# hypha-space/hypha

Hardware: AMD Instinct MI355X
Metric: tokens/sec (node) + outer-sync bytes, Llama-3-8B DiLoCo H=100 at 1/2/4/8 GPUs (higher is better)
Workload: dtype bf16; 1 GPU; model=llama3-8b, global_batch=8, seq_len=2048, parallelism=diloco-dp1, h=100, model_params=8030261248, memory_mode=full, outer_sync_payload_bytes=16060522496, outer_sync_wire_bytes_per_rank=0, comm_reduction_vs_ddp=100x fewer syncs, bf16 payload, native_ops=True

## Files before the change

hypha_amd/ops/hip/attention.hip:

```cpp

#include <climits>

#include <torch/extension.h>

#include "attn_tile.h"
#include "hip_common.h"

namespace {

typedef __attribute__((ext_vector_type(2))) __bf16 bf16x2;

template <int HD>
__global__ __launch_bounds__(256, 1) void attn_fwd_kernel(
    const short* __restrict__ qg, const short* __restrict__ kg,
    const short* __restrict__ vg, short* __restrict__ og, float* __restrict__ lseg,
    int B, int Hq, int Hkv, int S, float scale, bool causal,
    long long q_sb, long long q_sh, long long q_ss,
    long long kv_sb, long long kv_sh, long long kv_ss) {
  constexpr int KC = HD / 16;
  constexpr int DBLK = HD / 32;
  __shared__ __attribute__((aligned(16))) short k_lds[KVB * HD];
  __shared__ __attribute__((aligned(16))) short vt_lds[HD * VT_PITCH];
  __shared__ __attribute__((aligned(16))) short ot_lds[NWAVE][QB * (HD + 8)];

  const int tid = threadIdx.x;
  const int lane = tid & 63;
  const int wid = tid >> 6;
  const int hi = lane >> 5;
  const int ln = lane & 31;

  const int bh = blockIdx.y;
  const int b = bh / Hq;
  const int hq = bh % Hq;
  const int hkv = hq / (Hq / Hkv);
  const long long qbase = (long long)b * q_sb + (long long)hq * q_sh;
  const long long kvbase = (long long)b * kv_sb + (long long)hkv * kv_sh;

  const int q0wg = blockIdx.x * WGQ;
  const int q0 = q0wg + wid * QB;
  const int qrow = q0 + ln;
  const int vis = causal ? qrow : INT_MAX;

  s16x8 qfrag[KC];
// ... 58 lines not shown
    q_sh = HD; q_ss = (long long)Hq * HD; q_sb = (long long)S * Hq * HD;
    kv_sh = HD; kv_ss = (long long)Hkv * HD; kv_sb = (long long)S * Hkv * HD;
  } else {
    q_ss = HD; q_sh = (long long)S * HD; q_sb = (long long)Hq * S * HD;
    kv_ss = HD; kv_sh = (long long)S * HD; kv_sb = (long long)Hkv * S * HD;
  }
#define LAUNCH_FWD(HDV)                                                                 \
  hipLaunchKernelGGL(attn_fwd_kernel<HDV>, grid, dim3(256), 0, stream,                  \
                     (const short*)q.data_ptr(), (const short*)k.data_ptr(),            \
                     (const short*)v.data_ptr(), (short*)o.data_ptr(),                  \
                     lse.data_ptr<float>(), B, Hq, Hkv, S, scale, causal, q_sb, q_sh,   \
                     q_ss, kv_sb, kv_sh, kv_ss)
  if (HD == 128)
    LAUNCH_FWD(128);
  else
    LAUNCH_FWD(64);
#undef LAUNCH_FWD
  return {o, lse};
}

std::vector<torch::Tensor> attn_fwd(torch::Tensor q, torch::Tensor k, torch::Tensor v,
                                    bool causal) {
  return attn_fwd_ex(q, k, v, causal, "bhsd");
}


namespace {

template <int HD>
__global__ void attn_bwd_di_kernel(const short* __restrict__ dog,
                                   const short* __restrict__ og,
                                   float* __restrict__ dig, long long nrows, int Hq,
                                   int S, long long sb, long long sh, long long ss) {
  const long long row = (long long)blockIdx.x * 4 + (threadIdx.x >> 6);
  if (row >= nrows) return;
  const long long b = row / ((long long)Hq * S);
  const long long h = (row / S) % Hq;
  const long long sq = row % S;
  const long long addr = b * sb + h * sh + sq * ss;
  const int lane = threadIdx.x & 63;
  float acc = 0.f;
#pragma unroll
  for (int i = 0; i < HD / 64; ++i) {
    int d = lane + 64 * i;
    acc += bf2f(dog[addr + d]) * bf2f(og[addr + d]);
  }
  acc = wave_reduce_sum(acc);
  if (lane == 0) dig[row] = acc;
}

__global__ void cast_f32_to_bf16_kernel(const float* __restrict__ in,
                                        short* __restrict__ out, long long n) {
  const long long stride = (long long)gridDim.x * blockDim.x * 4;
  for (long long base = ((long long)blockIdx.x * blockDim.x + threadIdx.x) * 4; base < n;
       base += stride) {
    if (base + 4 <= n) {
      f32x4 v = *reinterpret_cast<const f32x4*>(in + base);
      s16x4 o;
#pragma unroll
      for (int j = 0; j < 4; ++j) o[j] = f2bf(v[j]);
      *reinterpret_cast<s16x4*>(out + base) = o;
    } else {
      for (long long i = base; i < n; ++i) out[i] = f2bf(in[i]);
    }
  }
}

template <int HD>
__global__ __launch_bounds__(256, 1) void attn_bwd_v4_kernel(
    const short* __restrict__ qg, const short* __restrict__ kg,
    const short* __restrict__ vg, const short* __restrict__ dog,
    const float* __restrict__ lseg, const float* __restrict__ dig,
    float* __restrict__ dqg, short* __restrict__ dkg, short* __restrict__ dvg,
    int B, int Hq, int Hkv, int S, float scale, bool causal,
    long long q_sb, long long q_sh, long long q_ss,
    long long kv_sb, long long kv_sh, long long kv_ss, int ablate,
    int dq_bf16) {
  constexpr int KVT = 32;
  constexpr int NT = 4;
  constexpr int KVW = NT * KVT;
  constexpr int QT = 32;
  constexpr int KC = HD / 16;
  constexpr int DBLK = HD / 32;
  constexpr int TP = 40;
  constexpr int DSP = KVW + 8;
  constexpr int KTP = KVW + 8;
  __shared__ __attribute__((aligned(16))) short k_img[KVW * HD];
  __shared__ __attribute__((aligned(16))) short v_img[KVW * HD];
  __shared__ __attribute__((aligned(16))) short kt_img[HD * KTP];
  __shared__ __attribute__((aligned(16))) short qt_img[HD * 32];
  __shared__ __attribute__((aligned(16))) short dot_img[HD * 32];
  __shared__ __attribute__((aligned(16))) short ptds_img[NWAVE][KVT * TP];
  __shared__ __attribute__((aligned(16))) short dst_img[NWAVE][KVT * TP];
  __shared__ __attribute__((aligned(16))) short ds_img[2][QT * DSP];

  const int tid = threadIdx.x;
  const int lane = tid & 63;
  const int wid = tid >> 6;
  const int hi = lane >> 5;
  const int ln = lane & 31;

  const int bhkv = blockIdx.y;
  const int b = bhkv / Hkv;
  const int hkv = bhkv % Hkv;
  const int G = Hq / Hkv;
  const int kv_base = blockIdx.x * KVW;
  const long long kvbase = (long long)b * kv_sb + (long long)hkv * kv_sh;

  auto qimg_off = [](int d, int qe) {
    return d * 32 + ((((qe >> 3) ^ ((d >> 2) & 3)) << 3) | (qe & 7));
  };

  {
    constexpr int CH = KVW * HD / 8;
    for (int c = tid; c < CH; c += 256) {
      int row = c / (HD / 8), e0 = (c % (HD / 8)) * 8;
      s16x8 k8 = *reinterpret_cast<const s16x8*>(kg + kvbase + (long long)(kv_base + row) * kv_ss + e0);
      *reinterpret_cast<s16x8*>((char*)k_img + k_lds_off<HD>(row, e0)) = k8;
      s16x8 v8 = *reinterpret_cast<const s16x8*>(vg + kvbase + (long long)(kv_base + row) * kv_ss + e0);
      *reinterpret_cast<s16x8*>((char*)v_img + k_lds_off<HD>(row, e0)) = v8;
    }
#pragma unroll
    for (int half = 0; half < KVW / 64; ++half) {
      for (int i = 0; i < HD / 32; ++i) {
        int kvr = (tid & 63) + 64 * half;
        int e0 = (i * 4 + (tid >> 6)) * 8;
        s16x8 k8 = *reinterpret_cast<const s16x8*>(kg + kvbase + (long long)(kv_base + kvr) * kv_ss + e0);
#pragma unroll
        for (int j = 0; j < 8; ++j) kt_img[(e0 + j) * KTP + kvr] = k8[j];
      }
    }
  }
  __syncthreads();

  f32x16 dk_acc[DBLK] = {};
  f32x16 dv_acc[DBLK] = {};

  short* ptds = ptds_img[wid];
  short* dst = dst_img[wid];
  const int kv0 = kv_base + wid * KVT;

  const int t0 = causal ? kv_base / QT : 0;
  const int Tq = S / QT;
  constexpr int NSTG = HD / 16 / NWAVE;

  int prev_q0 = -1, prev_na = 0, pbuf = 0;
  long long prev_qbase = 0;

  auto run_dq = [&](int buf) {
    if (wid >= DBLK || prev_q0 < 0) return;
    const int db = wid;
    const int kck_hi = 2 * prev_na;
    f32x16 dq = {};
    for (int kck = 0; kck < kck_hi; ++kck) {
      s16x8 af = *reinterpret_cast<const s16x8*>(ds_img[buf] + ln * DSP + 16 * kck + 8 * hi);
      s16x8 bf = *reinterpret_cast<const s16x8*>(kt_img + (32 * db + ln) * KTP +
                                                 16 * kck + 8 * hi);
      dq = __builtin_amdgcn_mfma_f32_32x32x16_bf16(af, bf, dq, 0, 0, 0);
    }
    if (!(ablate & 1)) {
      if (dq_bf16) {
#pragma unroll
        for (int r = 0; r < 16; ++r) {
          int qi = prev_q0 + (r & 3) + 8 * (r >> 2) + 4 * hi;
          float other = __shfl_xor(dq[r], 1, 64);
          if ((ln & 1) == 0) {
            bf16x2 pkt;
            pkt.x = (__bf16)dq[r];
            pkt.y = (__bf16)other;
            __builtin_amdgcn_global_atomic_fadd_v2bf16(
                reinterpret_cast<bf16x2*>(
                    reinterpret_cast<short*>(dqg) +
                    (prev_qbase + (long long)qi * q_ss + 32 * db + ln)),
                pkt);
          }
        }
      } else {
#pragma unroll
        for (int r = 0; r < 16; ++r) {
          int qi = prev_q0 + (r & 3) + 8 * (r >> 2) + 4 * hi;
          atomicAdd(dqg + (prev_qbase + (long long)qi * q_ss + 32 * db + ln), dq[r]);
        }
      }
    } else {
      asm volatile("" ::"v"(dq[0]));
    }
  };

  for (int hq = hkv * G; hq < (hkv + 1) * G; ++hq) {
    const long long qbase = (long long)b * q_sb + (long long)hq * q_sh;
    const long long lsebase = (long long)(b * Hq + hq) * S;

    s16x8 qreg[NSTG], doreg[NSTG];
    auto issue_prefetch = [&](int t) {
#pragma unroll
      for (int i = 0; i < NSTG; ++i) {
        int it = wid + NWAVE * i;
        int d0 = 8 * hi + 16 * it;
        qreg[i] = *reinterpret_cast<const s16x8*>(qg + qbase + (long long)(t * QT + ln) * q_ss + d0);
        doreg[i] = *reinterpret_cast<const s16x8*>(dog + qbase + (long long)(t * QT + ln) * q_ss + d0);
      }
    };
    issue_prefetch(t0);
    float lse = lseg[lsebase + t0 * QT + ln];
    float di = dig[lsebase + t0 * QT + ln];

    for (int t = t0; t < Tq; ++t) {
      const int q0 = t * QT;
      const int qrow = q0 + ln;

#pragma unroll
      for (int i = 0; i < NSTG; ++i) {
        int it = wid + NWAVE * i;
        int d0 = 8 * hi + 16 * it;
#pragma unroll
        for (int j = 0; j < 8; ++j) {
          qt_img[qimg_off(d0 + j, ln)] = qreg[i][j];
          dot_img[qimg_off(d0 + j, ln)] = doreg[i][j];
        }
      }
      __syncthreads();

      const float lse_cur = lse, di_cur = di;
      if (t + 1 < Tq) {
        issue_prefetch(t + 1);
        lse = lseg[lsebase + (t + 1) * QT + ln];
        di = dig[lsebase + (t + 1) * QT + ln];
      }

      const int na = causal ? min(NT, (q0 + QT - 1 - kv_base) / KVT + 1) : NT;
      const int cbuf = pbuf ^ 1;

      if (!(ablate & 2)) run_dq(pbuf);

      if (wid < na) {
        f32x16 st = {};
#pragma unroll
        for (int kc = 0; kc < KC; ++kc) {
          s16x8 qf = *reinterpret_cast<const s16x8*>(qg + qbase + (long long)qrow * q_ss +
                                                     16 * kc + 8 * hi);
          s16x8 kf = *reinterpret_cast<const s16x8*>(
              (char*)k_img + k_lds_off<HD>(wid * KVT + ln, 16 * kc + 8 * hi));
          st = __builtin_amdgcn_mfma_f32_32x32x16_bf16(kf, qf, st, 0, 0, 0);
        }
        f32x16 pt;
#pragma unroll
        for (int r = 0; r < 16; ++r) {
          int kv = kv0 + (r & 3) + 8 * (r >> 2) + 4 * hi;
          float pv = (ablate & 4) ? st[r] * scale : __expf(st[r] * scale - lse_cur);
          if (causal && kv > qrow) pv = 0.f;
          pt[r] = pv;
        }
#pragma unroll
        for (int r = 0; r < 16; ++r) {
          int kv = (r & 3) + 8 * (r >> 2) + 4 * hi;
          ptds[kv * TP + ln] = f2bf(pt[r]);
        }
#pragma unroll
        for (int db = 0; db < DBLK; ++db) {
#pragma unroll
          for (int kcq = 0; kcq < QT / 16; ++kcq) {
            s16x8 af = *reinterpret_cast<const s16x8*>(
                dot_img + qimg_off(32 * db + ln, 16 * kcq + 8 * hi));
            s16x8 bf = *reinterpret_cast<const s16x8*>(ptds + ln * TP + 16 * kcq + 8 * hi);
            dv_acc[db] = __builtin_amdgcn_mfma_f32_32x32x16_bf16(af, bf, dv_acc[db], 0, 0, 0);
          }
        }
        f32x16 dpt = {};
#pragma unroll
        for (int kc = 0; kc < KC; ++kc) {
          s16x8 df = *reinterpret_cast<const s16x8*>(dog + qbase + (long long)qrow * q_ss +
                                                     16 * kc + 8 * hi);
          s16x8 vf = *reinterpret_cast<const s16x8*>(
              (char*)v_img + k_lds_off<HD>(wid * KVT + ln, 16 * kc + 8 * hi));
          dpt = __builtin_amdgcn_mfma_f32_32x32x16_bf16(vf, df, dpt, 0, 0, 0);
        }
#pragma unroll
        for (int r = 0; r < 16; r += 2) {
          int kv = (r & 3) + 8 * (r >> 2) + 4 * hi;
          float v0 = pt[r] * (dpt[r] - di_cur) * scale;
          float v1 = pt[r + 1] * (dpt[r + 1] - di_cur) * scale;
          dst[kv * TP + ln] = f2bf(v0);
          dst[(kv + 1) * TP + ln] = f2bf(v1);
          *reinterpret_cast<unsigned*>(ds_img[cbuf] + ln * DSP + wid * KVT + kv) =
              pack_bf16x2(v0, v1);
        }
#pragma unroll
        for (int db = 0; db < DBLK; ++db) {
#pragma unroll
          for (int kcq = 0; kcq < QT / 16; ++kcq) {
            s16x8 af = *reinterpret_cast<const s16x8*>(dst + ln * TP + 16 * kcq + 8 * hi);
            s16x8 bf = *reinterpret_cast<const s16x8*>(
                qt_img + qimg_off(32 * db + ln, 16 * kcq + 8 * hi));
            dk_acc[db] = __builtin_amdgcn_mfma_f32_32x32x16_bf16(af, bf, dk_acc[db], 0, 0, 0);
          }
        }
      }
      __syncthreads();

      prev_q0 = q0;
      prev_na = na;
      prev_qbase = qbase;
      pbuf = cbuf;
    }
  }

  if (!(ablate & 2)) run_dq(pbuf);

#pragma unroll
  for (int db = 0; db < DBLK; ++db) {
#pragma unroll
    for (int r = 0; r < 16; ++r) {
      int m = (r & 3) + 8 * (r >> 2) + 4 * hi;
      dkg[kvbase + (long long)(kv0 + m) * kv_ss + 32 * db + ln] = f2bf(dk_acc[db][r]);
      dvg[kvbase + (long long)(kv0 + ln) * kv_ss + 32 * db + m] = f2bf(dv_acc[db][r]);
    }
  }
}

}

std::vector<torch::Tensor> attn_bwd_ex(torch::Tensor q, torch::Tensor k, torch::Tensor v,
                                       torch::Tensor o, torch::Tensor dout,
                                       torch::Tensor lse, bool causal,
                                       const std::string& layout) {
  auto bf16_dense = [](const torch::Tensor& t) {
    return t.is_cuda() && t.dim() == 4 && t.dtype() == torch::kBFloat16 &&
           t.is_contiguous();
  };
  TORCH_CHECK(bf16_dense(q), "attn_bwd: q must be a contiguous 4-D bf16 tensor");
  TORCH_CHECK(layout == "bhsd" || layout == "bshd",
              "attn_bwd: layout must be bhsd or bshd");
  const bool bshd = layout == "bshd";
  const int B = q.size(0);
  const int Hq = bshd ? q.size(2) : q.size(1);
  const int S = bshd ? q.size(1) : q.size(2);
  const int HD = q.size(3);
  TORCH_CHECK(bf16_dense(k) && k.size(0) == B && k.size(3) == HD &&
                  (bshd ? k.size(1) : k.size(2)) == S,
              "attn_bwd: k must be a contiguous bf16 tensor with q's batch, seq len "
              "and head dim");
  const int Hkv = bshd ? k.size(2) : k.size(1);
  TORCH_CHECK(Hkv > 0 && Hq % Hkv == 0, "attn_bwd: Hq must be a multiple of Hkv");
  TORCH_CHECK(bf16_dense(v) && v.sizes() == k.sizes(),
              "attn_bwd: v must be a contiguous bf16 tensor of k's shape");
  TORCH_CHECK(bf16_dense(o) && o.sizes() == q.sizes(),
              "attn_bwd: o must be a contiguous bf16 tensor of q's shape");
  TORCH_CHECK(bf16_dense(dout) && dout.sizes() == q.sizes(),
              "attn_bwd: dout must be a contiguous bf16 tensor of q's shape");
  TORCH_CHECK(lse.is_cuda() && lse.dtype() == torch::kFloat32 && lse.is_contiguous() &&
                  lse.numel() == (long long)B * Hq * S,
              "attn_bwd: lse must be a contiguous fp32 tensor of B*Hq*S elements");
  TORCH_CHECK(HD == 64 || HD == 128);
  TORCH_CHECK(S % 128 == 0, "seq len must be a multiple of 128");
  auto dk = torch::empty_like(k);
  auto dv = torch::empty_like(v);
  auto di = torch::empty({B, Hq, S}, q.options().dtype(torch::kFloat32));
  const float scale = 1.0f / sqrtf((float)HD);
  hipStream_t stream = hypha_stream();
  long long nrows = (long long)B * Hq * S;
  long long q_sb, q_sh, q_ss, kv_sb, kv_sh, kv_ss;
  if (bshd) {
    q_sh = HD; q_ss = (long long)Hq * HD; q_sb = (long long)S * Hq * HD;
    kv_sh = HD; kv_ss = (long long)Hkv * HD; kv_sb = (long long)S * Hkv * HD;
  } else {
    q_ss = HD; q_sh = (long long)S * HD; q_sb = (long long)Hq * S * HD;
    kv_ss = HD; kv_sh = (long long)S * HD; kv_sb = (long long)Hkv * S * HD;
  }

  static const int bwd_ablate = [] {
    const char* e = getenv("HYPHA_ATTN_ABLATE");
    return e ? atoi(e) : 0;
  }();
  static const bool dq_bf16 = [] {
    const char* e = getenv("HYPHA_ATTN_DQ_BF16");
    return e && e[0] == '1';
  }();
  auto dq32 = dq_bf16 ? torch::zeros(q.sizes(), q.options())
                      : torch::zeros(q.sizes(), q.options().dtype(torch::kFloat32));

#define DISPATCH(HDV)                                                                   \
  do {                                                                                  \
    hipLaunchKernelGGL(attn_bwd_di_kernel<HDV>, dim3((unsigned)((nrows + 3) / 4)),      \
                       dim3(256), 0, stream, (const short*)dout.data_ptr(),             \
                       (const short*)o.data_ptr(), di.data_ptr<float>(), nrows, Hq, S,  \
                       q_sb, q_sh, q_ss);                                               \
    hipLaunchKernelGGL(attn_bwd_v4_kernel<HDV>, dim3(S / 128, B * Hkv), dim3(256), 0,   \
                       stream, (const short*)q.data_ptr(), (const short*)k.data_ptr(),  \
                       (const short*)v.data_ptr(), (const short*)dout.data_ptr(),       \
                       lse.data_ptr<float>(), di.data_ptr<float>(),                     \
                       (float*)dq32.data_ptr(), (short*)dk.data_ptr(),                  \
                       (short*)dv.data_ptr(), B, Hq, Hkv, S, scale, causal, q_sb, q_sh, \
                       q_ss, kv_sb, kv_sh, kv_ss, bwd_ablate, dq_bf16 ? 1 : 0);         \
  } while (0)

  if (HD == 128)
    DISPATCH(128);
  else
    DISPATCH(64);
#undef DISPATCH

  if (dq_bf16) return {dq32, dk, dv};
  auto dq = torch::empty_like(q);
  long long n = dq32.numel();
  hipLaunchKernelGGL(cast_f32_to_bf16_kernel, dim3(elementwise_grid((n + 3) / 4)),
                     dim3(256), 0, stream, dq32.data_ptr<float>(), (short*)dq.data_ptr(),
                     n);
  return {dq, dk, dv};
}

std::vector<torch::Tensor> attn_bwd(torch::Tensor q, torch::Tensor k, torch::Tensor v,
                                    torch::Tensor o, torch::Tensor dout,
                                    torch::Tensor lse, bool causal) {
  return attn_bwd_ex(q, k, v, o, dout, lse, causal, "bhsd");
}
```

hypha_amd/ops/hip/bindings.cpp:

```cpp

#include <torch/extension.h>

#include <vector>

void adamw_step_(torch::Tensor master, torch::Tensor param, torch::Tensor grad,
                 torch::Tensor m, torch::Tensor v, double lr, double beta1, double beta2,
                 double eps, double wd, long step);
void nesterov_step_(torch::Tensor theta, torch::Tensor delta, torch::Tensor mom, double lr,
                    double mu);
void extract_delta(torch::Tensor master, torch::Tensor theta0, torch::Tensor out);
void adamw8_step_(torch::Tensor master, torch::Tensor param, torch::Tensor grad,
                  torch::Tensor m8, torch::Tensor v8, torch::Tensor m_scale,
                  torch::Tensor v_scale, double lr, double beta1, double beta2,
                  double eps, double wd, long step);
torch::Tensor swiglu_fwd(torch::Tensor gate, torch::Tensor up);
torch::Tensor grad_norm_sq(torch::Tensor x);
torch::Tensor grouped_gemm(torch::Tensor x, torch::Tensor w, torch::Tensor group_offsets);
void adamw8_lean_(torch::Tensor param, torch::Tensor grad, torch::Tensor m8,
                  torch::Tensor v8, torch::Tensor m_scale, torch::Tensor v_scale,
                  double lr, double beta1, double beta2, double eps, double wd,
                  long step, long seed);
void extract_delta_bf16(torch::Tensor theta_t, torch::Tensor theta0, torch::Tensor out);
void nesterov_bf16_(torch::Tensor theta, torch::Tensor delta, torch::Tensor mom,
                    double lr, double mu, long seed);
std::vector<torch::Tensor> swiglu_bwd(torch::Tensor dout, torch::Tensor gate,
                                      torch::Tensor up);
std::vector<torch::Tensor> layernorm_fwd(torch::Tensor x, torch::Tensor w,
                                         torch::Tensor b, double eps);
std::vector<torch::Tensor> layernorm_bwd(torch::Tensor dy, torch::Tensor x,
                                         torch::Tensor w, torch::Tensor mean,
                                         torch::Tensor rstd);
torch::Tensor gelu_fwd(torch::Tensor x);
torch::Tensor gelu_bwd(torch::Tensor dy, torch::Tensor x);
std::vector<torch::Tensor> rmsnorm_fwd(torch::Tensor x, torch::Tensor w, double eps);
std::vector<torch::Tensor> add_rmsnorm_fwd(torch::Tensor a, torch::Tensor b,
                                           torch::Tensor w, double eps);
std::vector<torch::Tensor> add_rmsnorm_bwd(torch::Tensor dy, torch::Tensor dh,
                                           torch::Tensor h, torch::Tensor w,
                                           torch::Tensor rstd);
std::vector<torch::Tensor> rmsnorm_bwd(torch::Tensor dy, torch::Tensor x, torch::Tensor w,
                                       torch::Tensor rstd);
std::vector<torch::Tensor> rope_fwd(torch::Tensor q, torch::Tensor k, torch::Tensor cos_t,
                                    torch::Tensor sin_t, bool inverse);
std::vector<torch::Tensor> rope_fwd_ex(torch::Tensor q, torch::Tensor k,
                                       torch::Tensor cos_t, torch::Tensor sin_t,
                                       bool inverse, const std::string& layout);
std::vector<torch::Tensor> ce_fwd(torch::Tensor logits, torch::Tensor targets);
torch::Tensor ce_bwd_(torch::Tensor logits, torch::Tensor targets, torch::Tensor lse,
                      double scale);
std::vector<torch::Tensor> attn_fwd(torch::Tensor q, torch::Tensor k, torch::Tensor v,
                                    bool causal);
std::vector<torch::Tensor> attn_bwd(torch::Tensor q, torch::Tensor k, torch::Tensor v,
                                    torch::Tensor o, torch::Tensor dout, torch::Tensor lse,
                                    bool causal);
std::vector<torch::Tensor> attn_fwd_ex(torch::Tensor q, torch::Tensor k, torch::Tensor v,
                                       bool causal, const std::string& layout);
std::vector<torch::Tensor> attn_bwd_ex(torch::Tensor q, torch::Tensor k, torch::Tensor v,
                                       torch::Tensor o, torch::Tensor dout,
                                       torch::Tensor lse, bool causal,
                                       const std::string& layout);
torch::Tensor mfma_probe_32x32x16(torch::Tensor a, torch::Tensor b);
torch::Tensor mfma_probe_16x16x32(torch::Tensor a, torch::Tensor b);
std::vector<torch::Tensor> fp8_cast_transpose(torch::Tensor x, torch::Tensor scale,
                                              torch::Tensor partials, long skip_t);
void fp8_scale_update_(torch::Tensor partials, torch::Tensor scale, double margin,
                       long n);
long long fp8_cast_grid_size(long long R, long long C);
void adamw8_fp8_lean_(torch::Tensor w8, torch::Tensor wscale, torch::Tensor grad,
                      torch::Tensor m8, torch::Tensor v8, torch::Tensor m_scale,
                      torch::Tensor v_scale, double lr, double beta1, double beta2,
                      double eps, double wd, long step, long seed);
void fp8_extract_delta(torch::Tensor w8, torch::Tensor wscale, torch::Tensor theta0,
                       torch::Tensor out);
void fp8_requant_(torch::Tensor theta, torch::Tensor w8, torch::Tensor wscale,
                  long seed);
std::vector<torch::Tensor> fp8_weight_cast_transpose(torch::Tensor w8s,
                                                     torch::Tensor wscale,
                                                     torch::Tensor scale,
                                                     torch::Tensor partials);
torch::Tensor attn_decode(torch::Tensor q, torch::Tensor kcache, torch::Tensor vcache,
                          long t);
torch::Tensor attn_decode_graph(torch::Tensor q, torch::Tensor kcache,
                                torch::Tensor vcache, torch::Tensor t_dev);
torch::Tensor attn_decode_fp8(torch::Tensor q, torch::Tensor kcache,
                              torch::Tensor vcache, torch::Tensor kscale,
                              torch::Tensor vscale, long t);
torch::Tensor attn_decode_fp8_graph(torch::Tensor q, torch::Tensor kcache,
                                    torch::Tensor vcache, torch::Tensor kscale,
                                    torch::Tensor vscale, torch::Tensor t_dev);
void kv_append_fp8_(torch::Tensor k, torch::Tensor v, torch::Tensor k8,
                    torch::Tensor v8, torch::Tensor kscale, torch::Tensor vscale,
                    torch::Tensor pos);
torch::Tensor attn_decode_varlen(torch::Tensor q, torch::Tensor kcache,
                                 torch::Tensor vcache, torch::Tensor lens, long max_len);
torch::Tensor attn_decode_varlen_fp8(torch::Tensor q, torch::Tensor kcache,
// ... 31 lines not shown
torch::Tensor skinny_gemm(torch::Tensor x, torch::Tensor w);
torch::Tensor sample_token(torch::Tensor logits, torch::Tensor u, torch::Tensor temperature,
                           torch::Tensor top_k, torch::Tensor top_p);
torch::Tensor philox_uniform(torch::Tensor seed, torch::Tensor step, long n);

PYBIND11_MODULE(TORCH_EXTENSION_NAME, m) {
  m.def("adamw_step_", &adamw_step_);
  m.def("nesterov_step_", &nesterov_step_);
  m.def("extract_delta", &extract_delta);
  m.def("adamw8_step_", &adamw8_step_);
  m.def("swiglu_fwd", &swiglu_fwd);
  m.def("grad_norm_sq", &grad_norm_sq);
  m.def("grouped_gemm", &grouped_gemm);
  m.def("adamw8_lean_", &adamw8_lean_);
  m.def("extract_delta_bf16", &extract_delta_bf16);
  m.def("nesterov_bf16_", &nesterov_bf16_);
  m.def("swiglu_bwd", &swiglu_bwd);
  m.def("rmsnorm_fwd", &rmsnorm_fwd);
  m.def("add_rmsnorm_fwd", &add_rmsnorm_fwd);
  m.def("add_rmsnorm_bwd", &add_rmsnorm_bwd);
  m.def("rmsnorm_bwd", &rmsnorm_bwd);
  m.def("layernorm_fwd", &layernorm_fwd);
  m.def("layernorm_bwd", &layernorm_bwd);
  m.def("gelu_fwd", &gelu_fwd);
  m.def("gelu_bwd", &gelu_bwd);
  m.def("rope_fwd", &rope_fwd);
  m.def("rope_fwd_ex", &rope_fwd_ex);
  m.def("ce_fwd", &ce_fwd);
  m.def("ce_bwd_", &ce_bwd_);
  m.def("attn_fwd", &attn_fwd);
  m.def("attn_bwd", &attn_bwd);
  m.def("attn_fwd_ex", &attn_fwd_ex);
  m.def("attn_bwd_ex", &attn_bwd_ex);
  m.def("mfma_probe_32x32x16", &mfma_probe_32x32x16);
  m.def("mfma_probe_16x16x32", &mfma_probe_16x16x32);
  m.def("fp8_cast_transpose", &fp8_cast_transpose, pybind11::arg("x"),
        pybind11::arg("scale"), pybind11::arg("partials"),
        pybind11::arg("skip_t") = 0);
  m.def("fp8_scale_update_", &fp8_scale_update_, pybind11::arg("partials"),
        pybind11::arg("scale"), pybind11::arg("margin"), pybind11::arg("n") = 0);
  m.def("fp8_cast_grid_size", &fp8_cast_grid_size);
  m.def("adamw8_fp8_lean_", &adamw8_fp8_lean_);
  m.def("fp8_extract_delta", &fp8_extract_delta);
  m.def("fp8_requant_", &fp8_requant_);
  m.def("fp8_weight_cast_transpose", &fp8_weight_cast_transpose);
  m.def("attn_decode", &attn_decode);
  m.def("attn_decode_graph", &attn_decode_graph);
  m.def("attn_decode_fp8", &attn_decode_fp8);
  m.def("attn_decode_fp8_graph", &attn_decode_fp8_graph);
  m.def("kv_append_fp8_", &kv_append_fp8_);
  m.def("attn_prefill", &attn_prefill);
  m.def("attn_prefill_fp8", &attn_prefill_fp8);
  m.def("attn_decode_varlen", &attn_decode_varlen);
  m.def("attn_decode_varlen_fp8", &attn_decode_varlen_fp8);
  m.def("kv_append_rows_", &kv_append_rows_);
  m.def("attn_prefill_varlen", &attn_prefill_varlen);
  m.def("attn_prefill_varlen_fp8", &attn_prefill_varlen_fp8);
  m.def("attn_decode_paged", &attn_decode_paged);
  m.def("attn_prefill_paged", &attn_prefill_paged);
  m.def("kv_append_paged_", &kv_append_paged_);
  m.def("skinny_gemm", &skinny_gemm);
  m.def("sample_token", &sample_token);
  m.def("philox_uniform", &philox_uniform);
}
```

hypha_amd/ops/hip/probe.hip:

```cpp

#include <torch/extension.h>

#include "hip_common.h"

__global__ void probe32_kernel(const short* __restrict__ a, const short* __restrict__ b,
                               float* __restrict__ d) {
  const int l = threadIdx.x;
  s16x8 af, bf;
#pragma unroll
  for (int j = 0; j < 8; ++j) {
    int k = 8 * (l >> 5) + j;
    af[j] = a[(l & 31) * 16 + k];
    bf[j] = b[k * 32 + (l & 31)];
  }
  f32x16 acc = {};
  acc = __builtin_amdgcn_mfma_f32_32x32x16_bf16(af, bf, acc, 0, 0, 0);
#pragma unroll
  for (int r = 0; r < 16; ++r) {
    int m = (r & 3) + 8 * (r >> 2) + 4 * (l >> 5);
    d[m * 32 + (l & 31)] = acc[r];
  }
}

__global__ void probe16_kernel(const short* __restrict__ a, const short* __restrict__ b,
                               float* __restrict__ d) {
  const int l = threadIdx.x;
  s16x8 af, bf;
#pragma unroll
  for (int j = 0; j < 8; ++j) {
    int k = 8 * (l >> 4) + j;
    af[j] = a[(l & 15) * 32 + k];
    bf[j] = b[k * 16 + (l & 15)];
  }
  f32x4 acc = {};
  acc = __builtin_amdgcn_mfma_f32_16x16x32_bf16(af, bf, acc, 0, 0, 0);
#pragma unroll
  for (int r = 0; r < 4; ++r) {
    int m = (l >> 4) * 4 + r;
    d[m * 16 + (l & 15)] = acc[r];
  }
}

torch::Tensor mfma_probe_32x32x16(torch::Tensor a, torch::Tensor b) {
  TORCH_CHECK(a.sizes() == torch::IntArrayRef({32, 16}) &&
              b.sizes() == torch::IntArrayRef({16, 32}));
  TORCH_CHECK(a.dtype() == torch::kBFloat16 && a.is_contiguous() && b.is_contiguous());
  auto d = torch::empty({32, 32}, a.options().dtype(torch::kFloat32));
  hipLaunchKernelGGL(probe32_kernel, dim3(1), dim3(64), 0, hypha_stream(),
                     (const short*)a.data_ptr(), (const short*)b.data_ptr(),
                     d.data_ptr<float>());
  return d;
}

torch::Tensor mfma_probe_16x16x32(torch::Tensor a, torch::Tensor b) {
  TORCH_CHECK(a.sizes() == torch::IntArrayRef({16, 32}) &&
              b.sizes() == torch::IntArrayRef({32, 16}));
  auto d = torch::empty({16, 16}, a.options().dtype(torch::kFloat32));
  hipLaunchKernelGGL(probe16_kernel, dim3(1), dim3(64), 0, hypha_stream(),
                     (const short*)a.data_ptr(), (const short*)b.data_ptr(),
                     d.data_ptr<float>());
  return d;
}
```

Baseline: 16960 tokens/s.

## Rewrite attention backward as key-lane kernel with transposed LDS reads

Replaces the v4 attention backward kernel with a key-lane kernel in which each wave owns 64 keys. V fragments stay in registers, Q/dO tiles are staged in swizzled, double-buffered LDS, and ds_read_tr16 transposed loads replace the explicit transposed K/Q/dO images. LSE and Di are folded into the MFMA accumulator initialisation, the grid is flattened with pair-major ordering, and the Di kernel is vectorised to 8-element loads. The goal is to cut LDS traffic, bank conflicts and register-to-LDS transposes in the backward pass, at the cost of higher register pressure and removal of the bf16 dq atomic option.

New measurement: 19170 tokens/s (median of 6 runs). 1.13x the previous value.

```diff
diff --git a/hypha_amd/ops/hip/attention.hip b/hypha_amd/ops/hip/attention.hip
--- a/hypha_amd/ops/hip/attention.hip
+++ b/hypha_amd/ops/hip/attention.hip
@@ -7,8 +7,6 @@
 #include "hip_common.h"
 
 namespace {
-
-typedef __attribute__((ext_vector_type(2))) __bf16 bf16x2;
 
 template <int HD>
 __global__ __launch_bounds__(256, 1) void attn_fwd_kernel(
@@ -133,21 +131,23 @@
                                    const short* __restrict__ og,
                                    float* __restrict__ dig, long long nrows, int Hq,
                                    int S, long long sb, long long sh, long long ss) {
-  const long long row = (long long)blockIdx.x * 4 + (threadIdx.x >> 6);
-  if (row >= nrows) return;
-  const long long b = row / ((long long)Hq * S);
-  const long long h = (row / S) % Hq;
-  const long long sq = row % S;
-  const long long addr = b * sb + h * sh + sq * ss;
-  const int lane = threadIdx.x & 63;
+  constexpr int LPR = HD / 8;
+  constexpr int RPB = 256 / LPR;
+  const long long row = (long long)blockIdx.x * RPB + threadIdx.x / LPR;
   float acc = 0.f;
-#pragma unroll
-  for (int i = 0; i < HD / 64; ++i) {
-    int d = lane + 64 * i;
-    acc += bf2f(dog[addr + d]) * bf2f(og[addr + d]);
-  }
-  acc = wave_reduce_sum(acc);
-  if (lane == 0) dig[row] = acc;
+  if (row < nrows) {
+    const long long b = row / ((long long)Hq * S);
+    const long long h = (row / S) % Hq;
+    const long long sq = row % S;
+    const long long addr = b * sb + h * sh + sq * ss + (threadIdx.x % LPR) * 8;
+    const s16x8 d8 = *reinterpret_cast<const s16x8*>(dog + addr);
+    const s16x8 o8 = *reinterpret_cast<const s16x8*>(og + addr);
+#pragma unroll
+    for (int j = 0; j < 8; ++j) acc += bf2f(d8[j]) * bf2f(o8[j]);
+  }
+#pragma unroll
+  for (int off = LPR / 2; off > 0; off >>= 1) acc += __shfl_xor(acc, off, 64);
+  if (row < nrows && threadIdx.x % LPR == 0) dig[row] = acc;
 }
 
 __global__ void cast_f32_to_bf16_kernel(const float* __restrict__ in,
@@ -168,121 +168,161 @@
 }
 
 template <int HD>
-__global__ __launch_bounds__(256, 1) void attn_bwd_v4_kernel(
+__device__ __forceinline__ int img_off(int row, int elem) {
+  const int ch = elem >> 3;
+  return (HD / 32) * 512 * (row >> 3) + 512 * (ch >> 2) + 64 * (row & 7) +
+         16 * ((ch & 3) ^ ((row >> 2) & 3)) + 2 * (elem & 7);
+}
+
+__device__ __forceinline__ int ds_off(int key, int unit) {
+  return key * 64 + ((unit ^ ((key >> 2) & 7)) << 3);
+}
+
+typedef __attribute__((address_space(3))) s16x4 lds_s16x4;
+
+__device__ __forceinline__ s16x8 lds_tr_pair(const short* img, int off0, int off1) {
+  s16x4 a = __builtin_amdgcn_ds_read_tr16_b64_v4i16((lds_s16x4*)((char*)img + off0));
+  s16x4 b = __builtin_amdgcn_ds_read_tr16_b64_v4i16((lds_s16x4*)((char*)img + off1));
+  return __builtin_shufflevector(a, b, 0, 1, 2, 3, 4, 5, 6, 7);
+}
+
+__device__ __forceinline__ s16x8 acc_frag(const f32x16& x, int s) {
+  unsigned w[4];
+#pragma unroll
+  for (int m = 0; m < 4; ++m) w[m] = pack_bf16x2(x[8 * s + 2 * m], x[8 * s + 2 * m + 1]);
+  return *reinterpret_cast<s16x8*>(w);
+}
+
+template <int HD, int KPW>
+__global__ __launch_bounds__(256, 1) void attn_bwd_keylane_kernel(
     const short* __restrict__ qg, const short* __restrict__ kg,
     const short* __restrict__ vg, const short* __restrict__ dog,
     const float* __restrict__ lseg, const float* __restrict__ dig,
     float* __restrict__ dqg, short* __restrict__ dkg, short* __restrict__ dvg,
     int B, int Hq, int Hkv, int S, float scale, bool causal,
     long long q_sb, long long q_sh, long long q_ss,
-    long long kv_sb, long long kv_sh, long long kv_ss, int ablate,
-    int dq_bf16) {
-  constexpr int KVT = 32;
-  constexpr int NT = 4;
-  constexpr int KVW = NT * KVT;
+    long long kv_sb, long long kv_sh, long long kv_ss, int ablate) {
+  constexpr int NH = KPW / 32;
+  constexpr int NT = NWAVE * NH;
+  constexpr int KVW = NWAVE * KPW;
   constexpr int QT = 32;
   constexpr int KC = HD / 16;
   constexpr int DBLK = HD / 32;
-  constexpr int TP = 40;
-  constexpr int DSP = KVW + 8;
-  constexpr int KTP = KVW + 8;
+  constexpr int NSTG = HD / 64;
   __shared__ __attribute__((aligned(16))) short k_img[KVW * HD];
-  __shared__ __attribute__((aligned(16))) short v_img[KVW * HD];
-  __shared__ __attribute__((aligned(16))) short kt_img[HD * KTP];
-  __shared__ __attribute__((aligned(16))) short qt_img[HD * 32];
-  __shared__ __attribute__((aligned(16))) short dot_img[HD * 32];
-  __shared__ __attribute__((aligned(16))) short ptds_img[NWAVE][KVT * TP];
-  __shared__ __attribute__((aligned(16))) short dst_img[NWAVE][KVT * TP];
-  __shared__ __attribute__((aligned(16))) short ds_img[2][QT * DSP];
+  __shared__ __attribute__((aligned(16))) short q_img[2][QT * HD];
+  __shared__ __attribute__((aligned(16))) short do_img[2][QT * HD];
+  __shared__ __attribute__((aligned(16))) short ds_img[2][KVW * QT];
+  __shared__ __attribute__((aligned(16))) float rc_img[2][2][QT];
 
   const int tid = threadIdx.x;
   const int lane = tid & 63;
-  const int wid = tid >> 6;
+  const int wid = __builtin_amdgcn_readfirstlane(tid >> 6);
   const int hi = lane >> 5;
   const int ln = lane & 31;
-
-  const int bhkv = blockIdx.y;
+  const int tg = (lane >> 4) & 1;
+  const int tq = (lane >> 2) & 3;
+  const int tp = lane & 3;
+
+  const int nkb = (S + KVW - 1) / KVW;
+  const int npair = B * Hkv;
+  int kb, bhkv;
+  if (ablate & 8) {
+    bhkv = blockIdx.x / nkb;
+    kb = blockIdx.x % nkb;
+  } else {
+    kb = blockIdx.x / npair;
+    bhkv = blockIdx.x % npair;
+  }
   const int b = bhkv / Hkv;
   const int hkv = bhkv % Hkv;
   const int G = Hq / Hkv;
-  const int kv_base = blockIdx.x * KVW;
+  const int kv_base = kb * KVW;
   const long long kvbase = (long long)b * kv_sb + (long long)hkv * kv_sh;
-
-  auto qimg_off = [](int d, int qe) {
-    return d * 32 + ((((qe >> 3) ^ ((d >> 2) & 3)) << 3) | (qe & 7));
+  const int nt_valid = min(NT, (S - kv_base) / 32);
+
+  for (int c = tid; c < KVW * HD / 8; c += 256) {
+    const int row = c / (HD / 8), e0 = (c % (HD / 8)) * 8;
+    s16x8 k8 = {};
+    if (kv_base + row < S)
+      k8 = *reinterpret_cast<const s16x8*>(kg + kvbase + (long long)(kv_base + row) * kv_ss + e0);
+    *reinterpret_cast<s16x8*>((char*)k_img + img_off<HD>(row, e0)) = k8;
+  }
+  s16x8 vfrag[NH][KC];
+#pragma unroll
+  for (int hh = 0; hh < NH; ++hh) {
+    const int key = kv_base + wid * KPW + 32 * hh + ln;
+#pragma unroll
+    for (int kc = 0; kc < KC; ++kc) {
+      s16x8 v8 = {};
+      if (key < S)
+        v8 = *reinterpret_cast<const s16x8*>(vg + kvbase + (long long)key * kv_ss + 16 * kc +
+                                             8 * hi);
+      vfrag[hh][kc] = v8;
+    }
+  }
+
+  f32x16 dk_acc[NH][DBLK] = {};
+  f32x16 dv_acc[NH][DBLK] = {};
+
+  const float c2 = 1.4426950408889634f * scale;
+  const float neg_sqrt_d = -1.0f / scale;
+  const int t0 = causal ? kv_base / QT : 0;
+  const int Tq = S / QT;
+
+  constexpr int GRP = (HD / 32) * 512;
+  int rd_base[2];
+#pragma unroll
+  for (int par = 0; par < 2; ++par)
+    rd_base[par] = GRP * (ln >> 3) + 64 * (ln & 7) + 16 * ((2 * par + hi) ^ ((ln >> 2) & 3));
+  auto rd = [&](const short* img, int kc) {
+    return *reinterpret_cast<const s16x8*>((const char*)img + rd_base[kc & 1] + 512 * (kc >> 1));
   };
-
-  {
-    constexpr int CH = KVW * HD / 8;
-    for (int c = tid; c < CH; c += 256) {
-      int row = c / (HD / 8), e0 = (c % (HD / 8)) * 8;
-      s16x8 k8 = *reinterpret_cast<const s16x8*>(kg + kvbase + (long long)(kv_base + row) * kv_ss + e0);
-      *reinterpret_cast<s16x8*>((char*)k_img + k_lds_off<HD>(row, e0)) = k8;
-      s16x8 v8 = *reinterpret_cast<const s16x8*>(vg + kvbase + (long long)(kv_base + row) * kv_ss + e0);
-      *reinterpret_cast<s16x8*>((char*)v_img + k_lds_off<HD>(row, e0)) = v8;
-    }
-#pragma unroll
-    for (int half = 0; half < KVW / 64; ++half) {
-      for (int i = 0; i < HD / 32; ++i) {
-        int kvr = (tid & 63) + 64 * half;
-        int e0 = (i * 4 + (tid >> 6)) * 8;
-        s16x8 k8 = *reinterpret_cast<const s16x8*>(kg + kvbase + (long long)(kv_base + kvr) * kv_ss + e0);
-#pragma unroll
-        for (int j = 0; j < 8; ++j) kt_img[(e0 + j) * KTP + kvr] = k8[j];
+  int tr_base[2];
+#pragma unroll
+  for (int x = 0; x < 2; ++x)
+    tr_base[x] = 64 * (4 * hi + tq) + 16 * ((2 * tg + (tp >> 1)) ^ (hi + 2 * x)) + 8 * (tp & 1);
+  auto tr_a = [&](const short* img, int db, int s) {
+    return lds_tr_pair(img, tr_base[0] + GRP * (2 * s) + 512 * db,
+                       tr_base[1] + GRP * (2 * s + 1) + 512 * db);
+  };
+  int trk_base[2], trs_base[2][2];
+#pragma unroll
+  for (int x = 0; x < 2; ++x) {
+    trk_base[x] = GRP * hi + 64 * (tq + 4 * x) + 16 * ((2 * tg + (tp >> 1)) ^ (2 * hi + x)) +
+                  8 * (tp & 1) + 512 * wid;
+#pragma unroll
+    for (int par = 0; par < 2; ++par)
+      trs_base[par][x] = 1024 * par + 64 * (8 * hi + tq + 4 * x) +
+                         8 * ((4 * tg + tp) ^ (4 * par + 2 * hi + x));
+  }
+
+  constexpr int RSTEP = 256 / (HD / 8);
+  const unsigned pf_off = (unsigned)(tid / (HD / 8)) * (unsigned)q_ss + (tid % (HD / 8)) * 8;
+
+  int prev_q0 = -1, prev_na = 0, buf = 0;
+  long long prev_qbase = 0;
+
+  auto run_dq = [&](int dbuf) {
+    if (wid >= DBLK || prev_q0 < 0) return;
+    const int db = wid;
+    f32x16 dq = {};
+    for (int kt = 0; kt < prev_na; ++kt) {
+#pragma unroll
+      for (int par = 0; par < 2; ++par) {
+        s16x8 af = lds_tr_pair(ds_img[dbuf], trs_base[par][0] + 2048 * kt,
+                               trs_base[par][1] + 2048 * kt);
+        s16x8 bf = lds_tr_pair(k_img, trk_base[0] + 2 * GRP * (2 * kt + par),
+                               trk_base[1] + 2 * GRP * (2 * kt + par));
+        dq = __builtin_amdgcn_mfma_f32_32x32x16_bf16(af, bf, dq, 0, 0, 0);
       }
     }
-  }
-  __syncthreads();
-
-  f32x16 dk_acc[DBLK] = {};
-  f32x16 dv_acc[DBLK] = {};
-
-  short* ptds = ptds_img[wid];
-  short* dst = dst_img[wid];
-  const int kv0 = kv_base + wid * KVT;
-
-  const int t0 = causal ? kv_base / QT : 0;
-  const int Tq = S / QT;
-  constexpr int NSTG = HD / 16 / NWAVE;
-
-  int prev_q0 = -1, prev_na = 0, pbuf = 0;
-  long long prev_qbase = 0;
-
-  auto run_dq = [&](int buf) {
-    if (wid >= DBLK || prev_q0 < 0) return;
-    const int db = wid;
-    const int kck_hi = 2 * prev_na;
-    f32x16 dq = {};
-    for (int kck = 0; kck < kck_hi; ++kck) {
-      s16x8 af = *reinterpret_cast<const s16x8*>(ds_img[buf] + ln * DSP + 16 * kck + 8 * hi);
-      s16x8 bf = *reinterpret_cast<const s16x8*>(kt_img + (32 * db + ln) * KTP +
-                                                 16 * kck + 8 * hi);
-      dq = __builtin_amdgcn_mfma_f32_32x32x16_bf16(af, bf, dq, 0, 0, 0);
-    }
     if (!(ablate & 1)) {
-      if (dq_bf16) {
-#pragma unroll
-        for (int r = 0; r < 16; ++r) {
-          int qi = prev_q0 + (r & 3) + 8 * (r >> 2) + 4 * hi;
-          float other = __shfl_xor(dq[r], 1, 64);
-          if ((ln & 1) == 0) {
-            bf16x2 pkt;
-            pkt.x = (__bf16)dq[r];
-            pkt.y = (__bf16)other;
-            __builtin_amdgcn_global_atomic_fadd_v2bf16(
-                reinterpret_cast<bf16x2*>(
-                    reinterpret_cast<short*>(dqg) +
-                    (prev_qbase + (long long)qi * q_ss + 32 * db + ln)),
-                pkt);
-          }
-        }
-      } else {
-#pragma unroll
-        for (int r = 0; r < 16; ++r) {
-          int qi = prev_q0 + (r & 3) + 8 * (r >> 2) + 4 * hi;
-          atomicAdd(dqg + (prev_qbase + (long long)qi * q_ss + 32 * db + ln), dq[r]);
-        }
-      }
+      float* tile = dqg + prev_qbase + (long long)prev_q0 * q_ss + 32 * db;
+      const unsigned voff = (unsigned)(4 * hi) * (unsigned)q_ss + ln;
+#pragma unroll
+      for (int r = 0; r < 16; ++r)
+        atomicAdd(tile + (long long)((r & 3) + 8 * (r >> 2)) * q_ss + voff, dq[r] * scale);
     } else {
       asm volatile("" ::"v"(dq[0]));
     }
@@ -293,138 +333,136 @@
     const long long lsebase = (long long)(b * Hq + hq) * S;
 
     s16x8 qreg[NSTG], doreg[NSTG];
+    float rcreg = 0.f;
     auto issue_prefetch = [&](int t) {
 #pragma unroll
       for (int i = 0; i < NSTG; ++i) {
-        int it = wid + NWAVE * i;
-        int d0 = 8 * hi + 16 * it;
-        qreg[i] = *reinterpret_cast<const s16x8*>(qg + qbase + (long long)(t * QT + ln) * q_ss + d0);
-        doreg[i] = *reinterpret_cast<const s16x8*>(dog + qbase + (long long)(t * QT + ln) * q_ss + d0);
+        const long long tile = qbase + (long long)(t * QT + RSTEP * i) * q_ss;
+        qreg[i] = *reinterpret_cast<const s16x8*>(qg + tile + pf_off);
+        doreg[i] = *reinterpret_cast<const s16x8*>(dog + tile + pf_off);
       }
+      if (wid == 0)
+        rcreg = hi ? -dig[lsebase + t * QT + ln] : lseg[lsebase + t * QT + ln] * neg_sqrt_d;
     };
     issue_prefetch(t0);
-    float lse = lseg[lsebase + t0 * QT + ln];
-    float di = dig[lsebase + t0 * QT + ln];
 
     for (int t = t0; t < Tq; ++t) {
       const int q0 = t * QT;
-      const int qrow = q0 + ln;
 
 #pragma unroll
       for (int i = 0; i < NSTG; ++i) {
-        int it = wid + NWAVE * i;
-        int d0 = 8 * hi + 16 * it;
-#pragma unroll
-        for (int j = 0; j < 8; ++j) {
-          qt_img[qimg_off(d0 + j, ln)] = qreg[i][j];
-          dot_img[qimg_off(d0 + j, ln)] = doreg[i][j];
-        }
+        const int c = tid + 256 * i;
+        const int off = img_off<HD>(c / (HD / 8), (c % (HD / 8)) * 8);
+        *reinterpret_cast<s16x8*>((char*)q_img[buf] + off) = qreg[i];
+        *reinterpret_cast<s16x8*>((char*)do_img[buf] + off) = doreg[i];
       }
+      if (wid == 0) rc_img[buf][hi][ln] = rcreg;
       __syncthreads();
 
-      const float lse_cur = lse, di_cur = di;
-      if (t + 1 < Tq) {
-        issue_prefetch(t + 1);
-        lse = lseg[lsebase + (t + 1) * QT + ln];
-        di = dig[lsebase + (t + 1) * QT + ln];
+      if (t + 1 < Tq) issue_prefetch(t + 1);
+
+      const int na = causal ? min(nt_valid, (q0 + QT - 1 - kv_base) / 32 + 1) : nt_valid;
+
+      if (!(ablate & 2)) run_dq(buf ^ 1);
+
+#pragma unroll
+      for (int hh = 0; hh < NH; ++hh) {
+        if (wid * NH + hh >= na) continue;
+        const int krow = wid * KPW + 32 * hh + ln;
+        const short* k_tile = k_img + (wid * KPW + 32 * hh) * HD;
+        const int key = kv_base + krow;
+        const bool diag = causal && kv_base + wid * KPW + 32 * hh + 31 > q0;
+
+        f32x16 s;
+#pragma unroll
+        for (int g = 0; g < 4; ++g) {
+          f32x4 c4 = *reinterpret_cast<const f32x4*>(&rc_img[buf][0][8 * g + 4 * hi]);
+#pragma unroll
+          for (int j = 0; j < 4; ++j) s[4 * g + j] = c4[j];
+        }
+#pragma unroll
+        for (int kc = 0; kc < KC; ++kc) {
+          s = __builtin_amdgcn_mfma_f32_32x32x16_bf16(rd(q_img[buf], kc), rd(k_tile, kc), s, 0, 0, 0);
+        }
+#pragma unroll
+        for (int r = 0; r < 16; ++r) {
+          float pv = (ablate & 4) ? s[r] * c2 : __builtin_amdgcn_exp2f(s[r] * c2);
+          if (diag && key > q0 + (r & 3) + 8 * (r >> 2) + 4 * hi) pv = 0.f;
+          s[r] = pv;
+        }
+        const s16x8 pf[2] = {acc_frag(s, 0), acc_frag(s, 1)};
+#pragma unroll
+        for (int db = 0; db < DBLK; ++db)
+#pragma unroll
+          for (int ks = 0; ks < 2; ++ks)
+            dv_acc[hh][db] = __builtin_amdgcn_mfma_f32_32x32x16_bf16(
+                tr_a(do_img[buf], db, ks), pf[ks], dv_acc[hh][db], 0, 0, 0);
+        f32x16 dp;
+#pragma unroll
+        for (int g = 0; g < 4; ++g) {
+          f32x4 c4 = *reinterpret_cast<const f32x4*>(&rc_img[buf][1][8 * g + 4 * hi]);
+#pragma unroll
+          for (int j = 0; j < 4; ++j) dp[4 * g + j] = c4[j];
+        }
+#pragma unroll
+        for (int kc = 0; kc < KC; ++kc) {
+          dp = __builtin_amdgcn_mfma_f32_32x32x16_bf16(rd(do_img[buf], kc), vfrag[hh][kc], dp, 0, 0, 0);
+        }
+#pragma unroll
+        for (int r = 0; r < 16; ++r) dp[r] *= s[r];
+        const s16x8 dsf[2] = {acc_frag(dp, 0), acc_frag(dp, 1)};
+#pragma unroll
+        for (int g = 0; g < 4; ++g) {
+          s16x4 d4 = (g & 1) ? __builtin_shufflevector(dsf[g >> 1], dsf[g >> 1], 4, 5, 6, 7)
+                             : __builtin_shufflevector(dsf[g >> 1], dsf[g >> 1], 0, 1, 2, 3);
+          *reinterpret_cast<s16x4*>((char*)ds_img[buf] + ds_off(krow, 2 * g + hi)) = d4;
+        }
+#pragma unroll
+        for (int db = 0; db < DBLK; ++db)
+#pragma unroll
+          for (int ks = 0; ks < 2; ++ks)
+            dk_acc[hh][db] = __builtin_amdgcn_mfma_f32_32x32x16_bf16(
+                tr_a(q_img[buf], db, ks), dsf[ks], dk_acc[hh][db], 0, 0, 0);
       }
-
-      const int na = causal ? min(NT, (q0 + QT - 1 - kv_base) / KVT + 1) : NT;
-      const int cbuf = pbuf ^ 1;
-
-      if (!(ablate & 2)) run_dq(pbuf);
-
-      if (wid < na) {
-        f32x16 st = {};
-#pragma unroll
-        for (int kc = 0; kc < KC; ++kc) {
-          s16x8 qf = *reinterpret_cast<const s16x8*>(qg + qbase + (long long)qrow * q_ss +
-                                                     16 * kc + 8 * hi);
-          s16x8 kf = *reinterpret_cast<const s16x8*>(
-              (char*)k_img + k_lds_off<HD>(wid * KVT + ln, 16 * kc + 8 * hi));
-          st = __builtin_amdgcn_mfma_f32_32x32x16_bf16(kf, qf, st, 0, 0, 0);
-        }
-        f32x16 pt;
-#pragma unroll
-        for (int r = 0; r < 16; ++r) {
-          int kv = kv0 + (r & 3) + 8 * (r >> 2) + 4 * hi;
-          float pv = (ablate & 4) ? st[r] * scale : __expf(st[r] * scale - lse_cur);
-          if (causal && kv > qrow) pv = 0.f;
-          pt[r] = pv;
-        }
-#pragma unroll
-        for (int r = 0; r < 16; ++r) {
-          int kv = (r & 3) + 8 * (r >> 2) + 4 * hi;
-          ptds[kv * TP + ln] = f2bf(pt[r]);
-        }
-#pragma unroll
-        for (int db = 0; db < DBLK; ++db) {
-#pragma unroll
-          for (int kcq = 0; kcq < QT / 16; ++kcq) {
-            s16x8 af = *reinterpret_cast<const s16x8*>(
-                dot_img + qimg_off(32 * db + ln, 16 * kcq + 8 * hi));
-            s16x8 bf = *reinterpret_cast<const s16x8*>(ptds + ln * TP + 16 * kcq + 8 * hi);
-            dv_acc[db] = __builtin_amdgcn_mfma_f32_32x32x16_bf16(af, bf, dv_acc[db], 0, 0, 0);
-          }
-        }
-        f32x16 dpt = {};
-#pragma unroll
-        for (int kc = 0; kc < KC; ++kc) {
-          s16x8 df = *reinterpret_cast<const s16x8*>(dog + qbase + (long long)qrow * q_ss +
-                                                     16 * kc + 8 * hi);
-          s16x8 vf = *reinterpret_cast<const s16x8*>(
-              (char*)v_img + k_lds_off<HD>(wid * KVT + ln, 16 * kc + 8 * hi));
-          dpt = __builtin_amdgcn_mfma_f32_32x32x16_bf16(vf, df, dpt, 0, 0, 0);
-        }
-#pragma unroll
-        for (int r = 0; r < 16; r += 2) {
-          int kv = (r & 3) + 8 * (r >> 2) + 4 * hi;
-          float v0 = pt[r] * (dpt[r] - di_cur) * scale;
-          float v1 = pt[r + 1] * (dpt[r + 1] - di_cur) * scale;
-          dst[kv * TP + ln] = f2bf(v0);
-          dst[(kv + 1) * TP + ln] = f2bf(v1);
-          *reinterpret_cast<unsigned*>(ds_img[cbuf] + ln * DSP + wid * KVT + kv) =
-              pack_bf16x2(v0, v1);
-        }
-#pragma unroll
-        for (int db = 0; db < DBLK; ++db) {
-#pragma unroll
-          for (int kcq = 0; kcq < QT / 16; ++kcq) {
-            s16x8 af = *reinterpret_cast<const s16x8*>(dst + ln * TP + 16 * kcq + 8 * hi);
-            s16x8 bf = *reinterpret_cast<const s16x8*>(
-                qt_img + qimg_off(32 * db + ln, 16 * kcq + 8 * hi));
-            dk_acc[db] = __builtin_amdgcn_mfma_f32_32x32x16_bf16(af, bf, dk_acc[db], 0, 0, 0);
-          }
-        }
-      }
-      __syncthreads();
 
       prev_q0 = q0;
       prev_na = na;
       prev_qbase = qbase;
-      pbuf = cbuf;
+      buf ^= 1;
     }
   }
 
-  if (!(ablate & 2)) run_dq(pbuf);
-
-#pragma unroll
-  for (int db = 0; db < DBLK; ++db) {
-#pragma unroll
-    for (int r = 0; r < 16; ++r) {
-      int m = (r & 3) + 8 * (r >> 2) + 4 * hi;
-      dkg[kvbase + (long long)(kv0 + m) * kv_ss + 32 * db + ln] = f2bf(dk_acc[db][r]);
-      dvg[kvbase + (long long)(kv0 + ln) * kv_ss + 32 * db + m] = f2bf(dv_acc[db][r]);
+  __syncthreads();
+  if (!(ablate & 2)) run_dq(buf ^ 1);
+
+#pragma unroll
+  for (int hh = 0; hh < NH; ++hh) {
+    if (wid * NH + hh >= nt_valid) continue;
+    const long long tile = kvbase + (long long)(kv_base + wid * KPW + 32 * hh) * kv_ss;
+    const unsigned voff = (unsigned)ln * (unsigned)kv_ss + 4 * hi;
+#pragma unroll
+    for (int db = 0; db < DBLK; ++db) {
+#pragma unroll
+      for (int g = 0; g < 4; ++g) {
+        s16x4 k4, v4;
+#pragma unroll
+        for (int j = 0; j < 4; ++j) {
+          k4[j] = f2bf(dk_acc[hh][db][4 * g + j] * scale);
+          v4[j] = f2bf(dv_acc[hh][db][4 * g + j]);
+        }
+        *reinterpret_cast<s16x4*>(dkg + tile + (32 * db + 8 * g) + voff) = k4;
+        *reinterpret_cast<s16x4*>(dvg + tile + (32 * db + 8 * g) + voff) = v4;
+      }
     }
   }
 }
 
 }
 
-std::vector<torch::Tensor> attn_bwd_ex(torch::Tensor q, torch::Tensor k, torch::Tensor v,
-                                       torch::Tensor o, torch::Tensor dout,
-                                       torch::Tensor lse, bool causal,
-                                       const std::string& layout) {
+void attn_bwd_into(torch::Tensor q, torch::Tensor k, torch::Tensor v, torch::Tensor o,
+                   torch::Tensor dout, torch::Tensor lse, bool causal,
+                   const std::string& layout, torch::Tensor dq, torch::Tensor dk,
+                   torch::Tensor dv) {
   auto bf16_dense = [](const torch::Tensor& t) {
     return t.is_cuda() && t.dim() == 4 && t.dtype() == torch::kBFloat16 &&
            t.is_contiguous();
@@ -454,8 +492,9 @@
               "attn_bwd: lse must be a contiguous fp32 tensor of B*Hq*S elements");
   TORCH_CHECK(HD == 64 || HD == 128);
   TORCH_CHECK(S % 128 == 0, "seq len must be a multiple of 128");
-  auto dk = torch::empty_like(k);
-  auto dv = torch::empty_like(v);
+  TORCH_CHECK(bf16_dense(dq) && dq.sizes() == q.sizes() && bf16_dense(dk) &&
+                  dk.sizes() == k.sizes() && bf16_dense(dv) && dv.sizes() == k.sizes(),
+              "attn_bwd: dq, dk, dv must be contiguous bf16 tensors of q's, k's and v's shapes");
   auto di = torch::empty({B, Hq, S}, q.options().dtype(torch::kFloat32));
   const float scale = 1.0f / sqrtf((float)HD);
   hipStream_t stream = hypha_stream();
@@ -473,26 +512,29 @@
     const char* e = getenv("HYPHA_ATTN_ABLATE");
     return e ? atoi(e) : 0;
   }();
-  static const bool dq_bf16 = [] {
-    const char* e = getenv("HYPHA_ATTN_DQ_BF16");
-    return e && e[0] == '1';
-  }();
-  auto dq32 = dq_bf16 ? torch::zeros(q.sizes(), q.options())
-                      : torch::zeros(q.sizes(), q.options().dtype(torch::kFloat32));
-
+  auto dq32 = torch::zeros(q.sizes(), q.options().dtype(torch::kFloat32));
+
+#define LAUNCH_BWD(HDV, KPWV)                                                           \
+  hipLaunchKernelGGL((attn_bwd_keylane_kernel<HDV, KPWV>),                              \
+                     dim3((unsigned)((S + 4 * KPWV - 1) / (4 * KPWV) * B * Hkv)),       \
+                     dim3(256), 0, stream, (const short*)q.data_ptr(),                  \
+                     (const short*)k.data_ptr(), (const short*)v.data_ptr(),            \
+                     (const short*)dout.data_ptr(), lse.data_ptr<float>(),              \
+                     di.data_ptr<float>(), dq32.data_ptr<float>(),                      \
+                     (short*)dk.data_ptr(), (short*)dv.data_ptr(), B, Hq, Hkv, S,       \
+                     scale, causal, q_sb, q_sh, q_ss, kv_sb, kv_sh, kv_ss, bwd_ablate)
 #define DISPATCH(HDV)                                                                   \
   do {                                                                                  \
-    hipLaunchKernelGGL(attn_bwd_di_kernel<HDV>, dim3((unsigned)((nrows + 3) / 4)),      \
+    constexpr int rows_per_block = 2048 / HDV;                                          \
+    hipLaunchKernelGGL(attn_bwd_di_kernel<HDV>,                                         \
+                       dim3((unsigned)((nrows + rows_per_block - 1) / rows_per_block)), \
                        dim3(256), 0, stream, (const short*)dout.data_ptr(),             \
                        (const short*)o.data_ptr(), di.data_ptr<float>(), nrows, Hq, S,  \
                        q_sb, q_sh, q_ss);                                               \
-    hipLaunchKernelGGL(attn_bwd_v4_kernel<HDV>, dim3(S / 128, B * Hkv), dim3(256), 0,   \
-                       stream, (const short*)q.data_ptr(), (const short*)k.data_ptr(),  \
-                       (const short*)v.data_ptr(), (const short*)dout.data_ptr(),       \
-                       lse.data_ptr<float>(), di.data_ptr<float>(),                     \
-                       (float*)dq32.data_ptr(), (short*)dk.data_ptr(),                  \
-                       (short*)dv.data_ptr(), B, Hq, Hkv, S, scale, causal, q_sb, q_sh, \
-                       q_ss, kv_sb, kv_sh, kv_ss, bwd_ablate, dq_bf16 ? 1 : 0);         \
+    if (bwd_ablate & 16)                                                                \
+      LAUNCH_BWD(HDV, 32);                                                              \
+    else                                                                                \
+      LAUNCH_BWD(HDV, 64);                                                              \
   } while (0)
 
   if (HD == 128)
@@ -500,13 +542,22 @@
   else
     DISPATCH(64);
 #undef DISPATCH
-
-  if (dq_bf16) return {dq32, dk, dv};
-  auto dq = torch::empty_like(q);
+#undef LAUNCH_BWD
+
   long long n = dq32.numel();
   hipLaunchKernelGGL(cast_f32_to_bf16_kernel, dim3(elementwise_grid((n + 3) / 4)),
                      dim3(256), 0, stream, dq32.data_ptr<float>(), (short*)dq.data_ptr(),
                      n);
+}
+
+std::vector<torch::Tensor> attn_bwd_ex(torch::Tensor q, torch::Tensor k, torch::Tensor v,
+                                       torch::Tensor o, torch::Tensor dout,
+                                       torch::Tensor lse, bool causal,
+                                       const std::string& layout) {
+  auto dq = torch::empty_like(q);
+  auto dk = torch::empty_like(k);
+  auto dv = torch::empty_like(v);
+  attn_bwd_into(q, k, v, o, dout, lse, causal, layout, dq, dk, dv);
   return {dq, dk, dv};
 }
 
diff --git a/hypha_amd/ops/hip/bindings.cpp b/hypha_amd/ops/hip/bindings.cpp
--- a/hypha_amd/ops/hip/bindings.cpp
+++ b/hypha_amd/ops/hip/bindings.cpp
@@ -55,12 +55,17 @@
                                     bool causal);
 std::vector<torch::Tensor> attn_fwd_ex(torch::Tensor q, torch::Tensor k, torch::Tensor v,
                                        bool causal, const std::string& layout);
+void attn_bwd_into(torch::Tensor q, torch::Tensor k, torch::Tensor v, torch::Tensor o,
+                   torch::Tensor dout, torch::Tensor lse, bool causal,
+                   const std::string& layout, torch::Tensor dq, torch::Tensor dk,
+                   torch::Tensor dv);
 std::vector<torch::Tensor> attn_bwd_ex(torch::Tensor q, torch::Tensor k, torch::Tensor v,
                                        torch::Tensor o, torch::Tensor dout,
                                        torch::Tensor lse, bool causal,
                                        const std::string& layout);
 torch::Tensor mfma_probe_32x32x16(torch::Tensor a, torch::Tensor b);
 torch::Tensor mfma_probe_16x16x32(torch::Tensor a, torch::Tensor b);
+torch::Tensor mfma_probe_acc_operand(torch::Tensor a, torch::Tensor m1, torch::Tensor m2);
 std::vector<torch::Tensor> fp8_cast_transpose(torch::Tensor x, torch::Tensor scale,
                                               torch::Tensor partials, long skip_t);
 void fp8_scale_update_(torch::Tensor partials, torch::Tensor scale, double margin,
@@ -158,8 +163,10 @@
   m.def("attn_bwd", &attn_bwd);
   m.def("attn_fwd_ex", &attn_fwd_ex);
   m.def("attn_bwd_ex", &attn_bwd_ex);
+  m.def("attn_bwd_into", &attn_bwd_into);
   m.def("mfma_probe_32x32x16", &mfma_probe_32x32x16);
   m.def("mfma_probe_16x16x32", &mfma_probe_16x16x32);
+  m.def("mfma_probe_acc_operand", &mfma_probe_acc_operand);
   m.def("fp8_cast_transpose", &fp8_cast_transpose, pybind11::arg("x"),
         pybind11::arg("scale"), pybind11::arg("partials"),
         pybind11::arg("skip_t") = 0);
diff --git a/hypha_amd/ops/hip/probe.hip b/hypha_amd/ops/hip/probe.hip
--- a/hypha_amd/ops/hip/probe.hip
+++ b/hypha_amd/ops/hip/probe.hip
@@ -41,6 +41,35 @@
   }
 }
 
+__global__ void probe_acc_operand_kernel(const short* __restrict__ a,
+                                         const short* __restrict__ m1,
+                                         const short* __restrict__ m2,
+                                         float* __restrict__ y) {
+  const int l = threadIdx.x;
+  const int h = l >> 5, n = l & 31;
+  s16x8 af, bf;
+#pragma unroll
+  for (int j = 0; j < 8; ++j) {
+    af[j] = m1[n * 16 + 8 * h + j];
+    bf[j] = m2[(8 * h + j) * 32 + n];
+  }
+  f32x16 x = {};
+  x = __builtin_amdgcn_mfma_f32_32x32x16_bf16(af, bf, x, 0, 0, 0);
+  f32x16 acc = {};
+#pragma unroll
+  for (int s = 0; s < 2; ++s) {
+    s16x8 xa, xb;
+#pragma unroll
+    for (int j = 0; j < 8; ++j) {
+      xb[j] = f2bf(x[8 * s + j]);
+      xa[j] = a[n * 32 + 16 * s + 8 * (j >> 2) + 4 * h + (j & 3)];
+    }
+    acc = __builtin_amdgcn_mfma_f32_32x32x16_bf16(xa, xb, acc, 0, 0, 0);
+  }
+#pragma unroll
+  for (int r = 0; r < 16; ++r) y[((r & 3) + 8 * (r >> 2) + 4 * h) * 32 + n] = acc[r];
+}
+
 torch::Tensor mfma_probe_32x32x16(torch::Tensor a, torch::Tensor b) {
   TORCH_CHECK(a.sizes() == torch::IntArrayRef({32, 16}) &&
               b.sizes() == torch::IntArrayRef({16, 32}));
@@ -61,3 +90,17 @@
                      d.data_ptr<float>());
   return d;
 }
+
+torch::Tensor mfma_probe_acc_operand(torch::Tensor a, torch::Tensor m1, torch::Tensor m2) {
+  auto ok = [](const torch::Tensor& t, int r, int c) {
+    return t.is_cuda() && t.dtype() == torch::kBFloat16 && t.is_contiguous() &&
+           t.sizes() == torch::IntArrayRef({r, c});
+  };
+  TORCH_CHECK(ok(a, 32, 32) && ok(m1, 32, 16) && ok(m2, 16, 32),
+              "mfma_probe_acc_operand: a [32,32], m1 [32,16], m2 [16,32], bf16 on the GPU");
+  auto y = torch::empty({32, 32}, a.options().dtype(torch::kFloat32));
+  hipLaunchKernelGGL(probe_acc_operand_kernel, dim3(1), dim3(64), 0, hypha_stream(),
+                     (const short*)a.data_ptr(), (const short*)m1.data_ptr(),
+                     (const short*)m2.data_ptr(), y.data_ptr<float>());
+  return y;
+}
```
